# KirillHit/snn_for_object_detection

Hardware: AMD Instinct MI355X
Metric: event-frames/sec (BxT) SODa-3M GEN1 304x240 fwd+bwd (higher is better)
Workload: dtype f32 (16-bit split products)

## Files before the change

include/snn_hip.h:

```cpp
#ifndef SNN_HIP_H
#define SNN_HIP_H

#include <stddef.h>
#include <stdint.h>

#ifdef __cplusplus
extern "C" {
#endif

#define SNN_ABI_VERSION 20

enum {
    SNN_NEURON_NONE = 0,
    SNN_NEURON_LIF = 1,
    SNN_NEURON_LI = 2,
    SNN_NEURON_LI_TANH = 3,
    SNN_NEURON_SLI = 4,
    SNN_NEURON_SYNAPSE = 5
};

enum { SNN_PREC_FP32 = 0, SNN_PREC_BF16X3 = 1, SNN_PREC_BF16X6 = 3, SNN_PREC_FP16X3 = 4, SNN_PREC_BF16X1 = 5,
       SNN_PREC_BF16S = 6 };

enum { SNN_SCAN_WIDE_ADDRESSING = 1,
// ... 95 lines not shown
int snn_conv2d_spikes_wgrad(const float* vdec, int64_t ld, float v_th, const float* dy, int64_t lddy, float* dw, int64_t N,
                            int H, int W, int Cin, int Ho, int Wo, int Cout, int KH, int KW, int stride, int pad,
                            int accumulate, float* workspace, int splitk, void* stream);
int snn_conv3x3_halo_spikes(const float* vdec, int64_t ld, float v_th, const void* w_image, float* y, int64_t ldy, int64_t N,
                            int H, int W, int Cin, int Cout, double* bn_partial, int frames_per_step, int* bn_layout,
                            void* stream);

int snn_conv1x1_mask_supported(int64_t N, int H, int W, int Cin, int Cout, const uint32_t* mask, int64_t ld_mask,
                               const float* w, const float* y, int64_t ldy, const float* dy, int64_t lddy, const float* dw,
                               int fwd_precision, int bwd_precision);
int snn_conv1x1_mask_fwd(const uint32_t* mask, int64_t ld_mask, const float* w, float* y, int64_t ldy, int64_t N, int H, int W,
                         int Cin, int Cout, void* stream);
int snn_conv1x1_mask_wgrad(const uint32_t* mask, int64_t ld_mask, const float* dy, int64_t lddy, float* dw, int64_t N, int H,
                           int W, int Cin, int Cout, int accumulate, float* workspace, int splitk, void* stream);

size_t snn_bn_stats_partial_size(int T, int64_t M, int C);
int snn_bn_stats(const float* y, int64_t ldy, int T, int64_t M, int C, double* partial, void* stream);
int snn_bn_stats_finalize(const double* partial, int chunks, int rows_per_chunk, int T, int64_t M, int C,
                          const float* gamma, const float* bias, float eps, float momentum,
                          float* running_mean, float* running_var, int use_running,
                          float* mean, float* invstd, float* alpha, float* beta, void* stream);

int snn_bn_stats_reduce(const double* partial, int chunks, int rows_per_chunk, int T, int64_t M, int C, double* sums,
                        void* stream);
int snn_bn_stats_from_sums(const double* sums, int T, int64_t M_total, int C,
                           const float* gamma, const float* bias, float eps, float momentum,
                           float* running_mean, float* running_var,
                           float* mean, float* invstd, float* alpha, float* beta,
                           double* var_scratch, void* stream);

// ... 278 lines not shown
```

snn_for_object_detection_amd/_hip.py:

```python

import ctypes
import os
from ctypes import POINTER, Structure, c_char_p, c_double, c_float, c_int, c_int32, c_int64, c_size_t, c_void_p

_HERE = os.path.dirname(os.path.abspath(__file__))
LIB_PATH = os.environ.get("SNN_HIP_LIB") or os.path.join(_HERE, "libsnn_hip.so")

NEURON_NONE, NEURON_LIF, NEURON_LI, NEURON_LI_TANH, NEURON_SLI, NEURON_SYNAPSE = 0, 1, 2, 3, 4, 5
POOL_AVG, POOL_MAX, POOL_SUM = 0, 1, 2
ACT_RELU, ACT_SILU, ACT_TANH = 0, 1, 2
ABI_VERSION = 20
PREC_FP32, PREC_BF16X3, PREC_BF16X6, PREC_FP16X3, PREC_BF16X1, PREC_BF16S = 0, 1, 3, 4, 5, 6
SCAN_WIDE_ADDRESSING, SCAN_LAST_STEP_ONLY, SCAN_BF16_STORAGE, SCAN_SPIKES_FROM_VDEC, SCAN_SUMS_FROM_STATE = 1, 2, 4, 8, 16
SCAN_STATE_LOOKBACK = 32
SCAN_SPIKE_MASK = 32
SURR_SUPER, SURR_TRIANGLE, SURR_SIGMOID, SURR_ATAN = 0, 1, 2, 3
ACTIVITY_NONZERO_F32, ACTIVITY_NONZERO_BF16, ACTIVITY_ABOVE_F32, ACTIVITY_ABOVE_BF16, ACTIVITY_MASK = 0, 1, 2, 3, 4
EVENT_REPS = {"binary": 0, "count": 1, "time": 2, "voxel": 3}
LOSS_CLS_MODES = {"ce": 0, "focal": 1}
LOSS_BOX_MODES = {"l1": 0, "giou": 1, "diou": 2, "ciou": 3}


class NeuronParams(Structure):
    _fields_ = [("c_mem", c_float), ("c_syn", c_float), ("v_leak", c_float), ("v_th", c_float),
# ... 36 lines not shown
    "snn_conv3x3_halo": (c_int, [_P, _L, _P, _P, _L, _L, _I, _I, _I, _I, _P, _L, _P, _L, _P, _I, _P, _I, _P]),
    "snn_conv2d_dgrad": (c_int, [_P, _L, _P, _P, _P, _L, _L, _I, _I, _I, _I, _I, _I, _I, _I, _I, _I, _P, _L, _P, _L,
                                 _I, _P]),
    "snn_conv2d_wgrad": (c_int, [_P, _L, _P, _L, _P, _L, _I, _I, _I, _I, _I, _I, _I, _I, _I, _I, _I, _P, _I, _I,
                                 _P]),
    "snn_conv2d_wgrad_splitk": (c_int, [_L, _I, _I, _I, _I, _I, _I, _I, _I, _I, _I, _I]),
    "snn_conv2d_wgrad_kernel": (c_int, [_L, _I, _I, _I, _I, _I, _I, _I, _I, _I, _I, _I]),
    "snn_conv2d_gather_plan": (c_int, [_I, _L, _I, _I, _I, _I, _I, _I, _I, _I, _I, _I, _L, _L, _I, _I, _I, _I, _I, _I, _I, _P]),
    "snn_conv2d_wgrad_plan": (c_int, [_L, _I, _I, _I, _I, _I, _I, _I, _I, _I, _I, _L, _L, _I, _I, _I, _I, _P]),
    "snn_conv1x1_spikes_supported": (c_int, [_L, _I, _I, _I, _I, _L, _I, _I]),
    "snn_conv1x1_spikes_fwd": (c_int, [_P, _L, _F, _P, _P, _L, _L, _I, _I, _I, _I, _P]),
    "snn_conv1x1_spikes_wgrad": (c_int, [_P, _L, _F, _P, _L, _P, _L, _I, _I, _I, _I, _I, _P, _I, _P]),
    "snn_conv1x1_mask_supported": (c_int, [_L, _I, _I, _I, _I, _P, _L, _P, _P, _L, _P, _L, _P, _I, _I]),
    "snn_conv1x1_mask_fwd": (c_int, [_P, _L, _P, _P, _L, _L, _I, _I, _I, _I, _P]),
    "snn_conv1x1_mask_wgrad": (c_int, [_P, _L, _P, _L, _P, _L, _I, _I, _I, _I, _I, _P, _I, _P]),
    "snn_conv2d_spikes_supported": (c_int, [_L, _I, _I, _I, _I, _I, _I, _I, _I, _I, _I, _L, _I, _I]),
    "snn_conv2d_spikes_fwd": (c_int, [_P, _L, _F, _P, _P, _L, _L, _I, _I, _I, _I, _I, _I, _I, _I, _I, _I, _P, _I, _P, _P]),
    "snn_conv2d_spikes_wgrad": (c_int, [_P, _L, _F, _P, _L, _P, _L, _I, _I, _I, _I, _I, _I, _I, _I, _I, _I, _I, _P, _I, _P]),
    "snn_conv3x3_halo_spikes": (c_int, [_P, _L, _F, _P, _P, _L, _L, _I, _I, _I, _I, _P, _I, _P, _P]),
    "snn_bn_stats_partial_size": (c_size_t, [_I, _L, _I]),
    "snn_bn_stats": (c_int, [_P, _L, _I, _L, _I, _P, _P]),
    "snn_bn_stats_finalize": (c_int, [_P, _I, _I, _I, _L, _I, _P, _P, _F, _F, _P, _P, _I, _P, _P, _P, _P, _P]),
    "snn_bn_stats_reduce": (c_int, [_P, _I, _I, _I, _L, _I, _P, _P]),
    "snn_bn_stats_from_sums": (c_int, [_P, _I, _L, _I, _P, _P, _F, _F, _P, _P, _P, _P, _P, _P, _P, _P]),
    "snn_bn_bwd_reduce": (c_int, [_P, _I, _L, _I, _P, _P]),
    "snn_bn_bwd_coef": (c_int, [_P, _P, _P, _I, _L, _I, _P, _P, _P, _P, _P, _P, _P, _P, _I, _P]),
    "snn_affine_neuron_fwd": (c_int, [_I, _P, _L, _P, _P, _P, _P, _P, _L, _P, _L, _P, _P, _P, _I, _L, _I,
                                      POINTER(NeuronParams), _I, _P]),
    "snn_affine_neuron_fwd_mask": (c_int, [_I, _P, _L, _P, _P, _P, _P, _P, _L, _P, _L, _P, _P, _P, _I, _L, _I,
                                           POINTER(NeuronParams), _I, _P, _P, _L]),
# ... 144 lines not shown
```

snn_for_object_detection_amd/csrc/conv_wgrad.hip:

```cpp
#include <stdlib.h>
#include <type_traits>
#include "conv_common.h"

namespace {

constexpr int WB_K = 32;

struct WgradGeom {
    int64_t Mtot;
    int H, W, Cin, Ho, Wo, Cout, KH, KW, stride, pad;
    int64_t ldx, lddy;
    int Ktot;
    int64_t pix_per_split;
    int tiles_m, tiles_n, splitk;
    int nimg;
    float x_th;
};

template <int TM, int TN, int WM, int WN, bool VEC>
__global__ __launch_bounds__(kThreads, SNN_CONV_MIN_WAVES) void k_conv_wgrad(const float* __restrict__ x, const float* __restrict__ dy,
                                                         float* __restrict__ ws, WgradGeom g) {
    static_assert(WM * WN == 4, "4 waves");
    constexpr int BMc = 32 * TM * WM, BNk = 32 * TN * WN;
    constexpr int DG = BMc / 4, XG = BNk / 4;
// ... 159 lines not shown
    float* slab = ws + (int64_t)z * g.Cout * (int64_t)g.Ktot;
#pragma unroll
    for (int i = 0; i < TM; ++i)
#pragma unroll
        for (int j = 0; j < TN; ++j) {
            const int kc = kc0 + (wn * TN + j) * 32 + r;
            if (kc >= g.Ktot) continue;
#pragma unroll
            for (int e = 0; e < 16; ++e) {
                const int co = co0 + (wm * TM + i) * 32 + (e & 3) + 8 * (e >> 2) + 4 * h;
                if (co < g.Cout) slab[(int64_t)co * g.Ktot + kc] = acc[i][j][e];
            }
        }
}

template <int TM, int TN, int WM, int WN, int WBK, bool ONE, bool SB = false, bool XSP = false, bool XM = false>
__global__ __launch_bounds__(kThreads, 2) void k_conv_wgrad_pipe(const float* __restrict__ x,
                                                                 const float* __restrict__ dy,
                                                                 float* __restrict__ ws, WgradGeom g) {
    static_assert(WM * WN == 4, "4 waves");
    constexpr int BMc = 32 * TM * WM, BNk = 32 * TN * WN;
    constexpr int DG = BMc / 4, XG = BNk / 4;
    static_assert(WBK == 32 || WBK == 64, "stage length");
    static_assert(!SB || ONE, "bf16 storage: one product");
    static_assert(!XSP || (!ONE && !SB), "spikes from potentials: the bf16 x 3 kernel");
    static_assert(!XM || XSP, "spike bit mask: an instance of the spikes-from-potentials kernel");
    constexpr int XW = ((BNk / 32) * WBK + kThreads - 1) / kThreads;
    constexpr int ES = SB ? 2 : 4;
    constexpr int LDW = WBK + 8;
    constexpr int NQ = WBK / 4;
    constexpr int GPP = kThreads / NQ;
    constexpr int DQ = (DG + GPP - 1) / GPP, XQ = (XG + GPP - 1) / GPP;
    __shared__ __attribute__((aligned(16))) __bf16 Dh[BMc * LDW];
    __shared__ __attribute__((aligned(16))) __bf16 Dl[ONE ? 8 : BMc * LDW];
    __shared__ __attribute__((aligned(16))) __bf16 Xh[XM ? 8 : BNk * LDW];
    __shared__ __attribute__((aligned(16))) __bf16 Xl[(ONE || XSP) ? 8 : BNk * LDW];
// ... 192 lines not shown
                for (int c = 0; c < 4; ++c) {
                    *reinterpret_cast<bf16x4*>(&Xh[(x_cq[q] + c) * LDW + quad * 4]) = px[q][c][0];
                    if constexpr (!ONE && !XSP) *reinterpret_cast<bf16x4*>(&Xl[(x_cq[q] + c) * LDW + quad * 4]) = px[q][c][1];
                }
            }
    };

    f32x16 acc[TM][TN];
#pragma unroll
    for (int i = 0; i < TM; ++i)
#pragma unroll
        for (int j = 0; j < TN; ++j)
#pragma unroll
            for (int e = 0; e < 16; ++e) acc[i][j][e] = 0.f;

    auto mfma_group = [&](int ks) {
        bf16x8 ah[TM], al[TM], bh[TN], bl[TN];
#pragma unroll
        for (int i = 0; i < TM; ++i) {
            const int off = ((wm * TM + i) * 32 + r) * LDW + ks * 16 + 8 * h;
            ah[i] = *reinterpret_cast<const bf16x8*>(&Dh[off]);
            if constexpr (!ONE) al[i] = *reinterpret_cast<const bf16x8*>(&Dl[off]);
        }
#pragma unroll
        for (int j = 0; j < TN; ++j) {
            if constexpr (XM) {
                const u32x4 w0 = *reinterpret_cast<const u32x4*>(&Xw[(wn * TN + j) * WBK + ks * 16 + 8 * h]);
                const u32x4 w1 = *reinterpret_cast<const u32x4*>(&Xw[(wn * TN + j) * WBK + ks * 16 + 8 * h + 4]);
                u32x4 d;
                d[0] = (((w0[0] >> r) & 1u) | (((w0[1] >> r) & 1u) << 16)) * 0x3F80u;
// ... 34 lines not shown
    for (int k = 0; k < XW; ++k) pxw[k] = rxw[k];
#pragma unroll
    for (int q = 0; q < XQ; ++q) {
        if constexpr (XM) continue;
        else if constexpr (XSP) convert_spikes(rx[q], px[q]);
        else convert_quad(rx[q], px[q]);
    }
    write_tiles();
    load_tiles(p_lo + WBK, 1);
    decode(0);
    __syncthreads();

    int slot = 0;
#pragma unroll 1
    for (unsigned p0 = p_lo; p0 < p_hi; p0 += WBK) {
        mfma_group(0);
#pragma unroll
        for (int q = 0; q < DQ; ++q) convert_quad(rd[q], pd[q]);
        __builtin_amdgcn_sched_group_barrier(0x100, NREAD, 0);
#pragma unroll
        for (int m = 0; m < NM; ++m) {
            __builtin_amdgcn_sched_group_barrier(0x008, 1, 0);
            __builtin_amdgcn_sched_group_barrier(0x002, VPG_D, 0);
        }
        __builtin_amdgcn_sched_barrier(0);
        mfma_group(1);
#pragma unroll
        for (int k = 0; k < XW; ++k) pxw[k] = rxw[k];
#pragma unroll
        for (int q = 0; q < XQ; ++q) {
            if constexpr (XM) continue;
            else if constexpr (XSP) convert_spikes(rx[q], px[q]);
            else convert_quad(rx[q], px[q]);
        }
        __builtin_amdgcn_sched_group_barrier(0x100, NREAD, 0);
#pragma unroll
        for (int m = 0; m < NM; ++m) {
            __builtin_amdgcn_sched_group_barrier(0x008, 1, 0);
            __builtin_amdgcn_sched_group_barrier(0x002, VPG_X, 0);
        }
        __builtin_amdgcn_sched_barrier(0);
#pragma unroll
        for (int ks = 2; ks < WBK / 16; ++ks) mfma_group(ks);
        load_tiles(p0 + 2 * WBK, slot);
        __syncthreads();
        write_tiles();
        decode(slot ^ 1);
        __syncthreads();
        slot ^= 1;
    }

    float* slab = ws + (int64_t)z * g.Cout * (int64_t)g.Ktot;
#pragma unroll
    for (int i = 0; i < TM; ++i)
#pragma unroll
        for (int j = 0; j < TN; ++j) {
            const int kcol = kc0 + (wn * TN + j) * 32 + r;
            if (kcol >= g.Ktot) continue;
// ... 392 lines not shown
    g.pix_per_split = p.pix_per_split;
    g.nimg = (int)N;
    g.tiles_m = p.tiles_m;
    g.tiles_n = p.tiles_n;
    g.splitk = splitk;
    dim3 grid((unsigned)((int64_t)g.tiles_m * g.tiles_n * splitk));
    hipStream_t st = (hipStream_t)stream;
    dispatch(
        [&](auto ID, auto KERNEL, auto WBK, auto ONE, auto SB, auto XSP, auto XM) {
            constexpr WgradShape t = kWgradShapes[ID()];
            if constexpr (KERNEL() != kWgradPipe) {
                hipLaunchKernelGGL((k_conv_wgrad<t.tm, t.tn, t.wm, t.wn, KERNEL() == kWgradVec>), grid, dim3(kThreads), 0, st, x, dy,
                                   workspace, g);
            } else if constexpr ((!SB() || ONE()) && (!XSP() || (!ONE() && !SB())) && (!XM() || XSP())) {
                hipLaunchKernelGGL((k_conv_wgrad_pipe<t.tm, t.tn, t.wm, t.wn, WBK(), ONE(), SB(), XSP(), XM()>), grid, dim3(kThreads), 0,
                                   st, x, dy, workspace, g);
            }
            return true;
        },
        OneOf<0, 1, 2, 3, 4, 5>{p.t.id}, OneOf<0, 1, 2>{p.kernel}, OneOf<32, 64>{p.wbk}, Flag{p.one}, Flag{sbf}, Flag{xsp}, Flag{xm});
    SNN_CHECK_LAUNCH("snn_conv2d_wgrad");
    return wgrad_reduce_slabs(workspace, dw, (int64_t)Cout * g.Ktot, splitk, accumulate, st);
}

extern "C" int snn_conv2d_wgrad_splitk(int64_t N, int H, int W, int Cin, int Ho, int Wo, int Cout, int KH, int KW,
                                       int stride, int pad, int precision) {
    if (N <= 0 || Ho <= 0 || Wo <= 0 || Cin <= 0 || Cout <= 0 || KH <= 0 || KW <= 0) return 1;
    return wgrad_plan(N, H, W, Cin, Ho, Wo, Cout, KH, KW, stride, pad, Cin, Cout, kAlignAll, precision, false, 0, 0).splitk;
}

extern "C" int snn_conv2d_wgrad_kernel(int64_t N, int H, int W, int Cin, int Ho, int Wo, int Cout, int KH, int KW, int stride,
// ... 88 lines not shown
        return false;
    const unsigned align = kAlignIn16 | kAlignDy16 | kAlignDy8 | (aligned(16, {dw}) ? kAlignDw16 : 0u);
    const WgradPlan p = wgrad_plan(N, H, W, Cin, H, W, Cout, 1, 1, 1, 0, ld_mask, lddy, align, SNN_PREC_BF16X3, true, 0, 0, false, true);
    return p.ok && p.kernel == kWgradPipe;
}

extern "C" int snn_conv1x1_mask_wgrad(const uint32_t* mask, int64_t ld_mask, const float* dy, int64_t lddy, float* dw, int64_t N,
                                      int H, int W, int Cin, int Cout, int accumulate, float* workspace, int splitk,
                                      void* stream) {
    SNN_REQUIRE(mask && dy && dw && workspace, "snn_conv1x1_mask_wgrad: null pointer");
    SNN_REQUIRE(snn_wgrad_mask_ok(N, H, W, Cin, Cout, mask, ld_mask, dy, lddy, dw),
                "snn_conv1x1_mask_wgrad: call not covered (ask snn_conv1x1_mask_supported)");
    return wgrad_common(reinterpret_cast<const float*>(mask), ld_mask, dy, lddy, dw, N, H, W, Cin, H, W, Cout, 1, 1, 1, 0,
                        accumulate, workspace, splitk, SNN_PREC_BF16X3, stream, true, 0.0f, true);
}
```

snn_for_object_detection_amd/functional.py:

```python

import collections
import contextlib
import ctypes
import functools
import os
import struct
from typing import List, NamedTuple, Optional, Sequence, Tuple

import torch
from torch.autograd import Function

from . import _hip
from ._hip import NeuronParams
from ._layout import (_BF16, _F32, ConcatPromise, Dest, _add_cl, _alias, _cl_view, _Convert, _copy_cl,
                      _dims5, _new_cl, _out_tensor, _ptr, _raw_convert, _raw_dense_cl, _raw_to_cl, _raw_to_nchw,
                      _require_device, _stream, _through_fp32, _ToChannelsLast, as_sequence, cl_stride, is_channels_last,
                      to_bfloat16, to_channels_last, to_float32)
from .pointwise import (POOL2D_COVERED, _Act, _Pool, _PoolPad, _SPP, _Upsample, activation, pool2d,
                        pool_covers, pool_sets, spp_covers, upsample_nearest)
from .losses import (MAX_LABEL_STEPS, _DetectionLoss, _GatherSteps, _loss_entry, _loss_ext, _require_steps,
                     check_loss_options, detection_loss, detection_loss_ext, detection_loss_steps,
                     detection_loss_steps_ext, gather_steps, select_label_steps)
from .event_ops import (AUG_Q16_MAX, AUG_Q16_MIN, AUG_Q16_ONE, _check_batch_vectors, _launch_batch_scatter,
                        check_aug_table, events_to_frames, events_to_frames_aug, events_to_frames_packed, labels_augment)

LEVERS = ("USE_WGRAD_STREAM", "USE_HEAD_STREAMS", "WGRAD_SIDE_DEPTH", "FUSE_OUTER_ADDEND", "USE_SIBLING_FUSION",
          "USE_SPIKES_FROM_VDEC", "USE_SPIKE_MASK", "SPIKE_MASK_MIN_BYTES", "USE_HALO_CONV", "USE_DEFERRED_BN_APPLY",
          "SCAN_SEGMENT_T", "USE_CONV_BN_STATS", "USE_PRESPLIT_WEIGHTS", "USE_PRESPLIT_DGRAD", "SCAN_FLAGS",
          "USE_SUMS_FROM_STATE", "LIF_CHECKPOINT_BYTES", "USE_LSTM_SCAN")


@contextlib.contextmanager
def levers(**values):
    unknown = sorted(set(values) - set(LEVERS))
    if unknown:
        raise AttributeError(f"functional has no lever {', '.join(unknown)} (LEVERS: {', '.join(LEVERS)})")
    found = {name: globals()[name] for name in values}
    globals().update(values)
    try:
        yield
    finally:
        globals().update(found)

DEFAULT_DT = 0.001
# ... 385 lines not shown
        self.result = dx


def _acc_of(x):
    return getattr(x, "_snn_acc", None)


def _same_tensor(a: torch.Tensor, b: torch.Tensor) -> bool:
    return (a.data_ptr() == b.data_ptr() and tuple(a.shape) == tuple(b.shape) and a.stride() == b.stride())


def _slot_of(param) -> Optional[GradSlot]:
    return getattr(param, "_snn_grad_slot", None) if param is not None else None


def _dgrad_accumulate(acc, gy, ldg, wt, x, geom, st, prec, wt_split=None, wt_image=None):
    T, B, Cin, H, W, Cout, KH, KW, Ho, Wo, stride, pad = geom
    dx, dx_shape = None, (T, B, Cin, H, W)
    addend, ld_add, addend2, ld_add2 = None, 0, None, 0
    outer_fused = None
    if acc is not None and acc[0].result is None and acc[0].deposits:
        key, other = next(iter(acc[0].deposits.items()))
        other = _raw_to_cl(other)
        if tuple(other.shape) == dx_shape:
            addend, ld_add = other.data_ptr(), cl_stride(other)
            acc[0].fused[key] = acc[0].deposits.pop(key)
    if (acc is not None and acc[0].result is None and not acc[0].deposits and acc[0].outer is not None
            and FUSE_OUTER_ADDEND):
        o_acc, o_key = acc[0].outer
        if o_acc.result is None and len(o_acc.deposits) == 1 and o_key not in o_acc.deposits:
            key2, other2 = next(iter(o_acc.deposits.items()))
            other2 = _raw_to_cl(other2)
            if tuple(other2.shape) == dx_shape:
                addend2, ld_add2 = other2.data_ptr(), cl_stride(other2)
                outer_fused = (o_acc, o_key, key2)
                if (o_acc.grad_in_slot and key2 in o_acc.exclusive and other2.dtype == x.dtype and ld_add2 % 4 == 0
                        and USE_SIBLING_FUSION):
                    dx = _alias(other2, other2.storage_offset(), T, B, Cin, H, W, ld_add2)
    chained = False
    if (acc is not None and acc[0].result is not None and addend is None and acc[1] not in acc[0].fused
            and tuple(acc[0].result.shape) == dx_shape):
        prev = acc[0].result
        addend, ld_add = prev.data_ptr(), cl_stride(prev)
        chained = True
    if dx is None:
        dx = _new_cl((T, B), Cin, H, W, x)
    if (prec in _HALO_BWD_PRECS and _halo_operand_ok(gy.data_ptr(), ldg, prec == _hip.PREC_BF16S) and USE_HALO_CONV
            and (KH, KW, stride, pad) == (3, 3, 2, 1)
            and _hip.query("snn_conv3x3_s2_dgrad_supported", T * B, H, W, Cin, Ho, Wo, Cout)):
        if wt_image is None:
            wt_image = _frag_image(wt, Cin, Cout, 1, _hip.PREC_BF16X3)
        _hip.call("snn_conv3x3_s2_dgrad", gy.data_ptr(), ldg, wt_image.data_ptr(), dx.data_ptr(), cl_stride(dx), T * B, H, W, Cin, Ho,
                  Wo, Cout, addend, ld_add, addend2, ld_add2, prec, st)
    elif (prec in _HALO_BWD_PRECS and _halo_operand_ok(gy.data_ptr(), ldg, prec == _hip.PREC_BF16S)
            and _halo_ok(T * B, H, W, Cout, Cin, KH, KW, stride, pad)):
        if wt_image is None:
            wt_image = _frag_image(wt, Cin, Cout, 1, _hip.PREC_BF16X3)
        _hip.call("snn_conv3x3_halo", gy.data_ptr(), ldg, wt_image.data_ptr(), dx.data_ptr(), cl_stride(dx), T * B, H, W, Cout,
                  Cin, addend, ld_add, addend2, ld_add2, None, 0, None, prec, st)
    else:
        _hip.call("snn_conv2d_dgrad", gy.data_ptr(), ldg, wt.data_ptr(), wt_split, dx.data_ptr(), cl_stride(dx), T * B, H, W,
                  Cin, Ho, Wo, Cout, KH, KW, stride, pad, addend, ld_add, addend2, ld_add2, prec, st)
    if acc is not None and (acc[0].result is None or chained):
        if chained and acc[0].outer is not None and acc[0].outer[0].result is acc[0].result:
            acc[0].outer[0].set_result(dx)
            acc[0].outer[0].fused[acc[0].outer[1]] = dx
        acc[0].set_result(dx)
        acc[0].fused[acc[1]] = dx
    if outer_fused is not None:
        o_acc, o_key, key2 = outer_fused
        o_acc.fused[key2] = o_acc.deposits.pop(key2)
        o_acc.fused[o_key] = dx
        o_acc.set_result(dx)
    return dx


USE_HALO_CONV = not os.environ.get("SNN_NO_HALO_CONV")
_HALO_BWD_PRECS = (_hip.PREC_BF16X3, _hip.PREC_BF16S)


def _halo_ok(N: int, H: int, W: int, Cin: int, Cout: int, KH: int, KW: int, stride: int, pad: int) -> bool:
    return (USE_HALO_CONV and KH == 3 and KW == 3 and stride == 1 and pad == 1
            and bool(_hip.query("snn_conv3x3_halo_supported", N, H, W, Cin, Cout)))


def _halo_operand_ok(ptr: int, ld: int, bf16: bool) -> bool:
    return ld % 4 == 0 and ptr % (8 if bf16 else 16) == 0


# ... 142 lines not shown
        dx = dw = None
        pend = _PENDING_APPLY.pop(gy.data_ptr(), None)
        if pend is not None:
            fused = (not ctx.needs_input_grad[0] and ctx.needs_input_grad[1] and ctx.slot is not None
                     and pend.gx.dtype == _F32 and pend.dims == (T, B, Cout, Ho, Wo) and cl_stride(pend.y) % 4 == 0
                     and _hip.query("snn_conv2d_wgrad_bn_supported", T * B, H, W, Cin, Ho, Wo, Cout, KH, KW, stride, pad))
            if fused:
                splitk = _hip.query("snn_conv2d_wgrad_splitk", T * B, H, W, Cin, Ho, Wo, Cout, KH, KW, stride, pad, ctx.prec)
                with _WgradLaunch(x.device, True, splitk, Cout, KH * KW * Cin,
                                   hold=(x, pend.gx, pend.y, pend.coef)) as (stream, ws, _):
                    _hip.call("snn_conv2d_wgrad_bn", x.data_ptr(), ldx, pend.gx.data_ptr(), Cout, pend.y.data_ptr(),
                              cl_stride(pend.y), pend.coef.data_ptr(), T, B, ctx.slot.buf.data_ptr(), T * B, H, W, Cin, Ho,
                              Wo, Cout, KH, KW, stride, pad, ctx.slot.claim(), ws.data_ptr(), splitk, stream)
                return None, None, None, None, None, None, None, None, None, None
            _apply_pending(pend)
        if ctx.needs_input_grad[0]:
            wt = _kept_view(ctx.weight, "_snn_wt")
            wt16 = wt_img = None
            if wt is not None:
                wt_img = _kept_view(ctx.weight, "_snn_wtfrag")
                if ctx.prec == _hip.PREC_BF16X3 and USE_PRESPLIT_WEIGHTS and USE_PRESPLIT_DGRAD:
                    wt16 = _ptr(_kept_view(ctx.weight, "_snn_wt16"))
            else:
                wt = torch.empty((Cin, KH, KW, Cout), device=x.device, dtype=_F32)
                _hip.call("snn_weight_transpose", w_ohwi.data_ptr(), wt.data_ptr(), Cout, KH, KW, Cin, st)
            dx = _dgrad_accumulate(ctx.acc, gy, ldg, wt, x, ctx.geom, st, ctx.prec, wt_split=wt16, wt_image=wt_img)
        if ctx.needs_input_grad[1]:
            splitk = _hip.query("snn_conv2d_wgrad_splitk", T * B, H, W, Cin, Ho, Wo, Cout, KH, KW, stride, pad, ctx.prec)
            xw, ldxw, x_th = _spikes_wgrad_operand(x, ldx, ctx.x_th, gy, ldg)
            slot = ctx.slot
            with _WgradLaunch(x.device, slot is not None, splitk, Cout, KH * KW * Cin,
                              hold=(x, xw, gy)) as (stream, ws, _):
                if slot is not None:
                    dst, accumulate = slot.buf, slot.claim()
                else:
                    dst, accumulate = torch.empty((Cout, KH, KW, Cin), device=x.device, dtype=_F32), 0
                if x_th is not None:
                    _hip.call("snn_conv2d_spikes_wgrad", xw.data_ptr(), ldxw, x_th, gy.data_ptr(), ldg, dst.data_ptr(),
                              T * B, H, W, Cin, Ho, Wo, Cout, KH, KW, stride, pad, accumulate, ws.data_ptr(), splitk,
                              stream)
                else:
                    _hip.call("snn_conv2d_wgrad", xw.data_ptr(), ldxw, gy.data_ptr(), ldg, dst.data_ptr(), T * B, H, W,
                              Cin, Ho, Wo, Cout, KH, KW, stride, pad, accumulate, ws.data_ptr(), splitk, ctx.prec,
                              stream)
            if slot is None:
                dw = dst.permute(0, 3, 1, 2)
        return dx, dw, None, None, None, None, None, None, None, None


def _small_gemm(a: torch.Tensor, trans_a: bool, b: torch.Tensor, trans_b: bool, c: torch.Tensor, accumulate: int,
                ct: Optional[torch.Tensor] = None, ct_col: int = 0) -> None:
    m, n = c.shape
# ... 144 lines not shown
        ctx.widths, ctx.c1 = widths, C1
        ctx.slot1, ctx.slots2 = slot1, slots2
        ctx.acc = acc
        return y

    @staticmethod
    def backward(ctx, gy):
        x, w1m, *w2ms = ctx.saved_tensors
        T, B, Cin, H, W, Ct = ctx.geom[:6]
        C1, widths = ctx.c1, ctx.widths
        composed = w1m is not None
        gy = _raw_to_cl(gy)
        ldg, ldx = cl_stride(gy), cl_stride(x)
        dx = dw1 = None
        dw2s = [None] * len(widths)
        if ctx.needs_input_grad[0]:
            dx = _dgrad_accumulate(ctx.acc, gy, ldg, ctx.wct, x, ctx.geom, _stream(), ctx.prec)
        if any(ctx.needs_input_grad[9:]) or (composed and ctx.needs_input_grad[1]):
            slot1, slots2 = ctx.slot1, ctx.slots2
            slotted = all(s_ is not None for s_ in slots2) and (slot1 is not None or not composed)
            splitk = _hip.query("snn_conv2d_wgrad_splitk", T * B, H, W, Cin, H, W, Ct, 1, 1, 1, 0, ctx.prec)
            xw, ldxw, x_th = _spikes_wgrad_operand(x, ldx, ctx.x_th, gy, ldg)
            x_mask = ctx.x_mask
            with _WgradLaunch(x.device, slotted, splitk, Ct, Cin, hold=(x, xw, gy, x_mask), with_g=True) as (stream, ws, G):
                if x_mask is not None and _hip.query("snn_conv1x1_mask_supported", T * B, H, W, Cin, Ct, x_mask.data_ptr(),
                                                     x_mask.shape[-1], None, None, 0, gy.data_ptr(), ldg, G.data_ptr(),
                                                     ctx.fwd_prec, ctx.prec):
                    _hip.call("snn_conv1x1_mask_wgrad", x_mask.data_ptr(), x_mask.shape[-1], gy.data_ptr(), ldg, G.data_ptr(),
                              T * B, H, W, Cin, Ct, 0, ws.data_ptr(), splitk, stream)
                elif x_th is not None:
                    _hip.call("snn_conv1x1_spikes_wgrad", xw.data_ptr(), ldxw, x_th, gy.data_ptr(), ldg, G.data_ptr(),
                              T * B, H, W, Cin, Ct, 0, ws.data_ptr(), splitk, stream)
                else:
                    _hip.call("snn_conv2d_wgrad", xw.data_ptr(), ldxw, gy.data_ptr(), ldg, G.data_ptr(), T * B, H, W,
                              Cin, H, W, Ct, 1, 1, 1, 0, 0, ws.data_ptr(), splitk, ctx.prec, stream)
                g1 = None
                if composed:
                    g1 = slot1.buf.view(C1, Cin) if slotted else torch.empty((C1, Cin), device=x.device, dtype=_F32)
                    acc1 = slot1.claim() if slotted else 0
                row = 0
                for b, (w2m, c) in enumerate(zip(w2ms, widths)):
                    Gb = G[row:row + c]
# ... 1139 lines not shown
```

snn_for_object_detection_amd/profiler.py:

```python

from collections import defaultdict
from typing import Dict

import torch


WGRAD_LABELS = ("k_conv_wgrad_pipe", "k_conv_wgrad_halo", "k_conv_first<wgrad>")


def _wgrad_label(n, h, w, cin, ho, wo, cout, kh, kw, stride, pad, prec) -> str:
    from . import _hip
    return WGRAD_LABELS[int(_hip.query("snn_conv2d_wgrad_kernel", n, h, w, cin, ho, wo, cout, kh, kw, stride, pad, prec))]


def _conv_label(name: str, a) -> str:
    if name == "snn_conv2d_wgrad":
        return _wgrad_label(a[5], a[6], a[7], a[8], a[9], a[10], a[11], a[12], a[13], a[14], a[15], a[19])
    dgrad = name == "snn_conv2d_dgrad"
    cin, cout = a[8], a[11]
    oc, ic = (cin, cout) if dgrad else (cout, cin)
    if not dgrad and cin == 2 and a[12] == 3 and a[13] == 3 and cout % 4 == 0 and (cout // 4) & (cout // 4 - 1) == 0 \
            and cout <= 256 and a[16] is None:
        return "k_conv_first<2, 3, false>"
    if oc <= 32:
# ... 31 lines not shown
        flops = 2.0 * n * h * w * cout * cin
        byts = 4.0 * (n * h * w * cin + n * h * w * cout + cout * cin)
        if not fwd:
            return WGRAD_LABELS[0], flops, byts
        tile = "32, 4, 1" if cout <= 32 else ("64, 2, 2" if cout <= 64 else "128, 2, 2")
        return f"k_conv_gather<{tile}, false, true>", flops, byts
    if name in ("snn_conv1x1_mask_fwd", "snn_conv1x1_mask_wgrad"):
        fwd = name.endswith("_fwd")
        n, h, w, cin, cout = (a[5], a[6], a[7], a[8], a[9])
        flops = 2.0 * n * h * w * cout * cin
        byts = n * h * w * cin / 8.0 + 4.0 * (n * h * w * cout + cout * cin)
        if not fwd:
            return WGRAD_LABELS[0] + ", mask, spikes", flops, byts
        tile = "32, 4, 1" if cout <= 32 else ("64, 2, 2" if cout <= 64 else "128, 2, 2")
        return f"k_conv_gather<{tile}, false, true>, mask, spikes", flops, byts
    if name in ("snn_conv2d_spikes_fwd", "snn_conv2d_spikes_wgrad"):
        fwd = name.endswith("_fwd")
        n, h, w, cin, ho, wo, cout, kh, kw, stride, pad = a[6:17]
        flops = 2.0 * n * ho * wo * cout * kh * kw * cin
        byts = 4.0 * (n * h * w * cin + n * ho * wo * cout + cout * kh * kw * cin)
        if not fwd:
            return _wgrad_label(n, h, w, cin, ho, wo, cout, kh, kw, stride, pad, 1) + ", spikes", flops, byts
        tile = "32, 4, 1" if cout <= 32 else ("64, 2, 2" if cout <= 64 else "128, 2, 2")
        return f"k_conv_gather<{tile}, false, true>", flops, byts
    if name == "snn_conv3x3_halo_spikes":
        n, h, w, cin, cout = a[6], a[7], a[8], a[9], a[10]
        flops = 2.0 * n * h * w * cout * 9 * cin
        byts = 4.0 * (n * h * w * cin + n * h * w * cout) + 4.0 * cout * 9 * cin
        return f"k_conv_halo3<{128 if cout % 128 == 0 else (64 if cout % 64 == 0 else 32)}, fwd, spikes>", flops, byts
    if name == "snn_conv3x3_halo":
# ... 123 lines not shown
```

Before: 7431.

## Fuse 1x1 conv data gradient into pipelined weight-gradient kernel

Adds a DX variant of the pipelined bf16x3 weight-gradient kernel. It reuses the dy tiles already staged in LDS (read transposed via ds_read_tr16) to compute dx for 1x1 convolutions, with the weights split into high and low bf16 parts held in registers, and it adds optional addends. The Python backward paths for plain and composed 1x1 convs route through this fused call when eligible, then run only a split-k reduce for dw. The goal is to avoid a separate dgrad pass that re-reads dy, at the cost of higher register pressure (launch bounds drop to 1 for some tiles) and extra MFMA work inside the wgrad loop.

New measurement: 7524, median of 6. 1.2% higher.

```diff
diff --git a/include/snn_hip.h b/include/snn_hip.h
--- a/include/snn_hip.h
+++ b/include/snn_hip.h
@@ -133,6 +133,20 @@
 int snn_conv1x1_mask_wgrad(const uint32_t* mask, int64_t ld_mask, const float* dy, int64_t lddy, float* dw, int64_t N, int H,
                            int W, int Cin, int Cout, int accumulate, float* workspace, int splitk, void* stream);
 
+int snn_conv1x1_bwd_supported(int64_t N, int H, int W, int Cin, int Cout, const void* x, int64_t ldx, int is_mask,
+                              const float* dy, int64_t lddy, const float* wt, const float* dx, int64_t lddx,
+                              const float* addend, int64_t ld_addend, const float* addend2, int64_t ld_addend2,
+                              const float* dw, int splitk, int precision);
+int snn_conv1x1_bwd(const float* x, int64_t ldx, const float* dy, int64_t lddy, const float* wt, float* dx, int64_t lddx,
+                    const float* addend, int64_t ld_addend, const float* addend2, int64_t ld_addend2, float* dw, int64_t N,
+                    int H, int W, int Cin, int Cout, int accumulate, float* workspace, int splitk, int precision,
+                    void* stream);
+int snn_conv1x1_mask_bwd(const uint32_t* mask, int64_t ld_mask, const float* dy, int64_t lddy, const float* wt, float* dx,
+                         int64_t lddx, const float* addend, int64_t ld_addend, const float* addend2, int64_t ld_addend2,
+                         float* dw, int64_t N, int H, int W, int Cin, int Cout, int accumulate, float* workspace, int splitk,
+                         int precision, void* stream);
+int snn_conv2d_wgrad_reduce(float* workspace, float* dw, int64_t n, int splitk, int accumulate, void* stream);
+
 size_t snn_bn_stats_partial_size(int T, int64_t M, int C);
 int snn_bn_stats(const float* y, int64_t ldy, int T, int64_t M, int C, double* partial, void* stream);
 int snn_bn_stats_finalize(const double* partial, int chunks, int rows_per_chunk, int T, int64_t M, int C,
diff --git a/snn_for_object_detection_amd/_hip.py b/snn_for_object_detection_amd/_hip.py
--- a/snn_for_object_detection_amd/_hip.py
+++ b/snn_for_object_detection_amd/_hip.py
@@ -74,6 +74,10 @@
     "snn_conv1x1_mask_supported": (c_int, [_L, _I, _I, _I, _I, _P, _L, _P, _P, _L, _P, _L, _P, _I, _I]),
     "snn_conv1x1_mask_fwd": (c_int, [_P, _L, _P, _P, _L, _L, _I, _I, _I, _I, _P]),
     "snn_conv1x1_mask_wgrad": (c_int, [_P, _L, _P, _L, _P, _L, _I, _I, _I, _I, _I, _P, _I, _P]),
+    "snn_conv1x1_bwd_supported": (c_int, [_L, _I, _I, _I, _I, _P, _L, _I, _P, _L, _P, _P, _L, _P, _L, _P, _L, _P, _I, _I]),
+    "snn_conv1x1_bwd": (c_int, [_P, _L, _P, _L, _P, _P, _L, _P, _L, _P, _L, _P, _L, _I, _I, _I, _I, _I, _P, _I, _I, _P]),
+    "snn_conv1x1_mask_bwd": (c_int, [_P, _L, _P, _L, _P, _P, _L, _P, _L, _P, _L, _P, _L, _I, _I, _I, _I, _I, _P, _I, _I, _P]),
+    "snn_conv2d_wgrad_reduce": (c_int, [_P, _P, _L, _I, _I, _P]),
     "snn_conv2d_spikes_supported": (c_int, [_L, _I, _I, _I, _I, _I, _I, _I, _I, _I, _I, _L, _I, _I]),
     "snn_conv2d_spikes_fwd": (c_int, [_P, _L, _F, _P, _P, _L, _L, _I, _I, _I, _I, _I, _I, _I, _I, _I, _I, _P, _I, _P, _P]),
     "snn_conv2d_spikes_wgrad": (c_int, [_P, _L, _F, _P, _L, _P, _L, _I, _I, _I, _I, _I, _I, _I, _I, _I, _I, _I, _P, _I, _P]),
diff --git a/snn_for_object_detection_amd/csrc/conv_wgrad.hip b/snn_for_object_detection_amd/csrc/conv_wgrad.hip
--- a/snn_for_object_detection_amd/csrc/conv_wgrad.hip
+++ b/snn_for_object_detection_amd/csrc/conv_wgrad.hip
@@ -197,12 +197,22 @@
         }
 }
 
-template <int TM, int TN, int WM, int WN, int WBK, bool ONE, bool SB = false, bool XSP = false, bool XM = false>
-__global__ __launch_bounds__(kThreads, 2) void k_conv_wgrad_pipe(const float* __restrict__ x,
+struct WgradDx {
+    const float* wt;
+    float* dx;
+    const float* add1;
+    const float* add2;
+    int64_t lddx, ld_add1, ld_add2;
+};
+typedef short s16x4 __attribute__((ext_vector_type(4)));
+template <int TM, int TN, int WM, int WN, int WBK, bool ONE, bool SB = false, bool XSP = false, bool XM = false, bool DX = false>
+__global__ __launch_bounds__(kThreads, (DX && TM * TN == 4 && !XM) ? 1 : 2) void k_conv_wgrad_pipe(const float* __restrict__ x,
                                                                  const float* __restrict__ dy,
-                                                                 float* __restrict__ ws, WgradGeom g) {
+                                                                 float* __restrict__ ws, WgradGeom g, WgradDx d) {
     static_assert(WM * WN == 4, "4 waves");
     constexpr int BMc = 32 * TM * WM, BNk = 32 * TN * WN;
+    static_assert(!DX || (!ONE && !SB && XSP == XM), "fused data gradient: bf16 x 3 on fp32 x or on the spike bit mask");
+    static_assert(!DX || (BNk / 32) * (WBK / 32) == 4, "fused data gradient: one 32 x 32 dx tile per wave and stage");
     constexpr int DG = BMc / 4, XG = BNk / 4;
     static_assert(WBK == 32 || WBK == 64, "stage length");
     static_assert(!SB || ONE, "bf16 storage: one product");
@@ -425,6 +435,36 @@
 #pragma unroll
             for (int e = 0; e < 16; ++e) acc[i][j][e] = 0.f;
 
+    constexpr int NCH = BMc / 16;
+    [[maybe_unused]] bf16x8 wh[DX ? NCH : 1], wl[DX ? NCH : 1];
+    [[maybe_unused]] const int dx_cg = wave % (BNk / 32), dx_pg = wave / (BNk / 32);
+    [[maybe_unused]] int dx_tr = 0;
+    if constexpr (DX) {
+        const int ci = kc0 + dx_cg * 32 + r;
+#pragma unroll
+        for (int c = 0; c < NCH; ++c) {
+            const int co = 16 * c + 8 * h;
+            f32x4 v[2] = {{0.f, 0.f, 0.f, 0.f}, {0.f, 0.f, 0.f, 0.f}};
+            if (ci < g.Cin) {
+                if (co < g.Cout) v[0] = *reinterpret_cast<const f32x4*>(d.wt + (int64_t)ci * g.Cout + co);
+                if (co + 4 < g.Cout) v[1] = *reinterpret_cast<const f32x4*>(d.wt + (int64_t)ci * g.Cout + co + 4);
+            }
+#pragma unroll
+            for (int e = 0; e < 8; e += 2) {
+                f32x2 rest = {v[e >> 2][e & 3], v[e >> 2][(e & 3) + 1]};
+                bf16x2 pp = __builtin_convertvector(rest, bf16x2);
+                const unsigned bits = __builtin_bit_cast(unsigned, pp);
+                wh[c][e] = pp[0]; wh[c][e + 1] = pp[1];
+                rest[0] -= __builtin_bit_cast(float, bits << 16);
+                rest[1] -= __builtin_bit_cast(float, bits & 0xffff0000u);
+                pp = __builtin_convertvector(rest, bf16x2);
+                wl[c][e] = pp[0]; wl[c][e + 1] = pp[1];
+            }
+        }
+        const int grp = lane_id >> 4, i16 = lane_id & 15;
+        dx_tr = (8 * (grp >> 1) + (i16 >> 2)) * LDW + dx_pg * 32 + 16 * (grp & 1) + 4 * (i16 & 3);
+    }
+
     auto mfma_group = [&](int ks) {
         bf16x8 ah[TM], al[TM], bh[TN], bl[TN];
 #pragma unroll
@@ -489,6 +529,18 @@
     int slot = 0;
 #pragma unroll 1
     for (unsigned p0 = p_lo; p0 < p_hi; p0 += WBK) {
+        [[maybe_unused]] f32x4 ad1[4], ad2[4];
+        [[maybe_unused]] const unsigned dx_p = p0 + (unsigned)(dx_pg * 32 + r);
+        [[maybe_unused]] const int dx_ci = kc0 + dx_cg * 32 + 4 * h;
+        if constexpr (DX) {
+#pragma unroll
+            for (int jj = 0; jj < 4; ++jj) {
+                const bool ok = dx_p < p_hi && dx_ci + 8 * jj < g.Cin;
+                ad1[jj] = ad2[jj] = f32x4{0.f, 0.f, 0.f, 0.f};
+                if (d.add1 && ok) ad1[jj] = SnnStore<false>::ld4_last(d.add1, (int64_t)dx_p * d.ld_add1 + dx_ci + 8 * jj);
+                if (d.add2 && ok) ad2[jj] = SnnStore<false>::ld4_last(d.add2, (int64_t)dx_p * d.ld_add2 + dx_ci + 8 * jj);
+            }
+        }
         mfma_group(0);
 #pragma unroll
         for (int q = 0; q < DQ; ++q) convert_quad(rd[q], pd[q]);
@@ -517,6 +569,33 @@
         __builtin_amdgcn_sched_barrier(0);
 #pragma unroll
         for (int ks = 2; ks < WBK / 16; ++ks) mfma_group(ks);
+        if constexpr (DX) {
+            f32x16 dacc;
+#pragma unroll
+            for (int e = 0; e < 16; ++e) dacc[e] = 0.f;
+            typedef __attribute__((address_space(3))) s16x4* LdsQuad;
+#pragma unroll
+            for (int c = 0; c < NCH; ++c) {
+                const int o = dx_tr + 16 * c * LDW;
+                const s16x4 h0 = __builtin_amdgcn_ds_read_tr16_b64_v4i16((LdsQuad)&Dh[o]);
+                const s16x4 h1 = __builtin_amdgcn_ds_read_tr16_b64_v4i16((LdsQuad)&Dh[o + 4 * LDW]);
+                const s16x4 l0 = __builtin_amdgcn_ds_read_tr16_b64_v4i16((LdsQuad)&Dl[o]);
+                const s16x4 l1 = __builtin_amdgcn_ds_read_tr16_b64_v4i16((LdsQuad)&Dl[o + 4 * LDW]);
+                const bf16x8 dh = __builtin_bit_cast(bf16x8, __builtin_shufflevector(h0, h1, 0, 1, 2, 3, 4, 5, 6, 7));
+                const bf16x8 dl = __builtin_bit_cast(bf16x8, __builtin_shufflevector(l0, l1, 0, 1, 2, 3, 4, 5, 6, 7));
+                dacc = __builtin_amdgcn_mfma_f32_32x32x16_bf16(wh[c], dl, dacc, 0, 0, 0);
+                dacc = __builtin_amdgcn_mfma_f32_32x32x16_bf16(wl[c], dh, dacc, 0, 0, 0);
+                dacc = __builtin_amdgcn_mfma_f32_32x32x16_bf16(wh[c], dh, dacc, 0, 0, 0);
+            }
+#pragma unroll
+            for (int jj = 0; jj < 4; ++jj) {
+                if (!(dx_p < p_hi && dx_ci + 8 * jj < g.Cin)) continue;
+                f32x4 v = {dacc[4 * jj], dacc[4 * jj + 1], dacc[4 * jj + 2], dacc[4 * jj + 3]};
+                if (d.add1) v += ad1[jj];
+                if (d.add2) v += ad2[jj];
+                SnnStore<false>::st4(d.dx, (int64_t)dx_p * d.lddx + dx_ci + 8 * jj, v);
+            }
+        }
         load_tiles(p0 + 2 * WBK, slot);
         __syncthreads();
         write_tiles();
@@ -939,7 +1018,7 @@
                                    workspace, g);
             } else if constexpr ((!SB() || ONE()) && (!XSP() || (!ONE() && !SB())) && (!XM() || XSP())) {
                 hipLaunchKernelGGL((k_conv_wgrad_pipe<t.tm, t.tn, t.wm, t.wn, WBK(), ONE(), SB(), XSP(), XM()>), grid, dim3(kThreads), 0,
-                                   st, x, dy, workspace, g);
+                                   st, x, dy, workspace, g, WgradDx{});
             }
             return true;
         },
@@ -1058,3 +1137,116 @@
     return wgrad_common(reinterpret_cast<const float*>(mask), ld_mask, dy, lddy, dw, N, H, W, Cin, H, W, Cout, 1, 1, 1, 0,
                         accumulate, workspace, splitk, SNN_PREC_BF16X3, stream, true, 0.0f, true);
 }
+
+namespace {
+struct Bwd1x1Call {
+    const void* x;
+    int64_t ldx;
+    bool xm;
+    const float* dy;
+    int64_t lddy;
+    const float* wt;
+    const float* dx;
+    int64_t lddx;
+    const float *add1, *add2;
+    int64_t ld_add1, ld_add2;
+    const float* dw;
+};
+static const char* bwd1x1_refusal(int64_t N, int H, int W, int Cin, int Cout, const Bwd1x1Call& c, int splitk, int precision,
+                                  WgradPlan* out) {
+    if (!(N > 0 && H > 0 && W > 0 && Cin > 0 && Cout > 0)) return "bad shape";
+    if (!(c.x && c.dy && c.wt && c.dx)) return "null pointer";
+    if (precision != SNN_PREC_BF16X3) return "bf16 x 3 arithmetic on fp32 tensors only";
+    if (Cout > 128) return "more than 128 output channels (a block must own all of them)";
+    if (Cout % 4 || Cin % 4) return "channel counts must be multiples of 4";
+    if (splitk < 0 || splitk > 32768) return "bad splitk";
+    if (c.xm ? !(Cin % 32 == 0 && c.ldx >= Cin / 32) : !(c.ldx >= Cin && c.ldx % 4 == 0))
+        return "x: pixel stride smaller than the channel count or no multiple of 4 (mask: Cin % 32, ld >= Cin / 32)";
+    if (!(c.lddy >= Cout && c.lddy % 4 == 0 && c.lddx >= Cin && c.lddx % 4 == 0))
+        return "dy / dx: pixel stride smaller than the channel count or no multiple of 4";
+    if (!(aligned(c.xm ? 4 : 16, {c.x}) && aligned(16, {c.dy, c.wt, c.dx}))) return "x, dy, wt and dx must be 16-byte aligned (mask: 4)";
+    if (c.add1 && !(c.ld_add1 >= Cin && c.ld_add1 % 4 == 0 && aligned(16, {c.add1}))) return "addend: stride or alignment";
+    if (c.add2 && !(c.ld_add2 >= Cin && c.ld_add2 % 4 == 0 && aligned(16, {c.add2}))) return "addend2: stride or alignment";
+    if (c.dw && !aligned(4, {c.dw})) return "dw must be 4-byte aligned";
+    if (!(N * H * (int64_t)W < 0x7fffffffLL - 64)) return "more than 2^31 pixels";
+    const unsigned align = kAlignIn16 | kAlignDy16 | kAlignDy8 | ((c.dw && aligned(16, {c.dw})) ? kAlignDw16 : 0u);
+    const WgradPlan p = wgrad_plan(N, H, W, Cin, H, W, Cout, 1, 1, 1, 0, c.ldx, c.lddy, align, precision, c.xm, 0, splitk, false, c.xm);
+    if (!(p.ok && p.kernel == kWgradPipe && !p.one)) return "the weight gradient does not take the pipelined bf16 x 3 kernel";
+    if (p.tiles_m != 1) return "the weight-gradient tile does not own all output channels";
+    if (!(p.t.id == 0 || p.t.id == 4)) return "no fused instance for this weight-gradient tile";
+    if (out) *out = p;
+    return nullptr;
+}
+
+static bool bwd1x1_pays(const WgradPlan& p, bool xm) {
+    return !(p.t.id == 0 && !xm);
+}
+
+static int bwd1x1_common(const char* name, const Bwd1x1Call& c, float* dx, float* dw, int64_t N, int H, int W, int Cin, int Cout,
+                         int accumulate, float* workspace, int splitk, int precision, void* stream) {
+    SNN_REQUIRE(workspace, "%s: null workspace", name);
+    SNN_REQUIRE(splitk >= 1, "%s: bad splitk %d", name, splitk);
+    WgradPlan p;
+    const char* why = bwd1x1_refusal(N, H, W, Cin, Cout, c, splitk, precision, &p);
+    SNN_REQUIRE(!why, "%s: call not covered: %s (ask snn_conv1x1_bwd_supported)", name, why);
+    WgradGeom g;
+    g.Mtot = N * H * (int64_t)W;
+    g.H = H; g.W = W; g.Cin = Cin; g.Ho = H; g.Wo = W; g.Cout = Cout;
+    g.KH = 1; g.KW = 1; g.stride = 1; g.pad = 0;
+    g.ldx = c.ldx; g.lddy = c.lddy;
+    g.Ktot = Cin;
+    g.x_th = 0.0f;
+    g.pix_per_split = p.pix_per_split;
+    g.nimg = (int)N;
+    g.tiles_m = p.tiles_m;
+    g.tiles_n = p.tiles_n;
+    g.splitk = splitk;
+    const WgradDx d = {c.wt, dx, c.add1, c.add2, c.lddx, c.ld_add1, c.ld_add2};
+    const dim3 grid((unsigned)((int64_t)g.tiles_m * g.tiles_n * splitk));
+    hipStream_t st = (hipStream_t)stream;
+    const float* xf = static_cast<const float*>(c.x);
+    dispatch(
+        [&](auto ID, auto XM) {
+            constexpr WgradShape t = kWgradShapes[ID()];
+            constexpr int wbk = ID() >= 4 ? 64 : 32;
+            hipLaunchKernelGGL((k_conv_wgrad_pipe<t.tm, t.tn, t.wm, t.wn, wbk, false, false, XM(), XM(), true>), grid, dim3(kThreads), 0, st,
+                               xf, c.dy, workspace, g, d);
+            return true;
+        },
+        OneOf<0, 4>{p.t.id}, Flag{c.xm});
+    SNN_CHECK_LAUNCH(name);
+    if (!dw) return 0;
+    return wgrad_reduce_slabs(workspace, dw, (int64_t)Cout * Cin, splitk, accumulate, st);
+}
+}
+
+extern "C" int snn_conv1x1_bwd_supported(int64_t N, int H, int W, int Cin, int Cout, const void* x, int64_t ldx, int is_mask,
+                                         const float* dy, int64_t lddy, const float* wt, const float* dx, int64_t lddx,
+                                         const float* addend, int64_t ld_addend, const float* addend2, int64_t ld_addend2,
+                                         const float* dw, int splitk, int precision) {
+    const Bwd1x1Call c = {x, ldx, is_mask != 0, dy, lddy, wt, dx, lddx, addend, addend2, ld_addend, ld_addend2, dw};
+    WgradPlan p;
+    if (bwd1x1_refusal(N, H, W, Cin, Cout, c, splitk, precision, &p)) return 0;
+    return bwd1x1_pays(p, c.xm) ? 1 : 0;
+}
+
+extern "C" int snn_conv1x1_bwd(const float* x, int64_t ldx, const float* dy, int64_t lddy, const float* wt, float* dx, int64_t lddx,
+                               const float* addend, int64_t ld_addend, const float* addend2, int64_t ld_addend2, float* dw,
+                               int64_t N, int H, int W, int Cin, int Cout, int accumulate, float* workspace, int splitk,
+                               int precision, void* stream) {
+    const Bwd1x1Call c = {x, ldx, false, dy, lddy, wt, dx, lddx, addend, addend2, ld_addend, ld_addend2, dw};
+    return bwd1x1_common("snn_conv1x1_bwd", c, dx, dw, N, H, W, Cin, Cout, accumulate, workspace, splitk, precision, stream);
+}
+
+extern "C" int snn_conv1x1_mask_bwd(const uint32_t* mask, int64_t ld_mask, const float* dy, int64_t lddy, const float* wt, float* dx,
+                                    int64_t lddx, const float* addend, int64_t ld_addend, const float* addend2,
+                                    int64_t ld_addend2, float* dw, int64_t N, int H, int W, int Cin, int Cout, int accumulate,
+                                    float* workspace, int splitk, int precision, void* stream) {
+    const Bwd1x1Call c = {mask, ld_mask, true, dy, lddy, wt, dx, lddx, addend, addend2, ld_addend, ld_addend2, dw};
+    return bwd1x1_common("snn_conv1x1_mask_bwd", c, dx, dw, N, H, W, Cin, Cout, accumulate, workspace, splitk, precision, stream);
+}
+
+extern "C" int snn_conv2d_wgrad_reduce(float* workspace, float* dw, int64_t n, int splitk, int accumulate, void* stream) {
+    SNN_REQUIRE(workspace && dw && n > 0 && splitk >= 1 && splitk <= 32768, "snn_conv2d_wgrad_reduce: bad arguments");
+    return wgrad_reduce_slabs(workspace, dw, n, splitk, accumulate, (hipStream_t)stream);
+}
diff --git a/snn_for_object_detection_amd/functional.py b/snn_for_object_detection_amd/functional.py
--- a/snn_for_object_detection_amd/functional.py
+++ b/snn_for_object_detection_amd/functional.py
@@ -27,7 +27,8 @@
 LEVERS = ("USE_WGRAD_STREAM", "USE_HEAD_STREAMS", "WGRAD_SIDE_DEPTH", "FUSE_OUTER_ADDEND", "USE_SIBLING_FUSION",
           "USE_SPIKES_FROM_VDEC", "USE_SPIKE_MASK", "SPIKE_MASK_MIN_BYTES", "USE_HALO_CONV", "USE_DEFERRED_BN_APPLY",
           "SCAN_SEGMENT_T", "USE_CONV_BN_STATS", "USE_PRESPLIT_WEIGHTS", "USE_PRESPLIT_DGRAD", "SCAN_FLAGS",
-          "USE_SUMS_FROM_STATE", "LIF_CHECKPOINT_BYTES", "USE_LSTM_SCAN")
+          "USE_SUMS_FROM_STATE", "LIF_CHECKPOINT_BYTES", "USE_LSTM_SCAN", "USE_FUSED_BWD1X1",
+          "FUSED_BWD1X1_MIN_BYTES")
 
 
 @contextlib.contextmanager
@@ -443,7 +444,7 @@
     return getattr(param, "_snn_grad_slot", None) if param is not None else None
 
 
-def _dgrad_accumulate(acc, gy, ldg, wt, x, geom, st, prec, wt_split=None, wt_image=None):
+def _dgrad_accumulate(acc, gy, ldg, wt, x, geom, st, prec, wt_split=None, wt_image=None, fuse=None):
     T, B, Cin, H, W, Cout, KH, KW, Ho, Wo, stride, pad = geom
     dx, dx_shape = None, (T, B, Cin, H, W)
     addend, ld_add, addend2, ld_add2 = None, 0, None, 0
@@ -474,7 +475,9 @@
         chained = True
     if dx is None:
         dx = _new_cl((T, B), Cin, H, W, x)
-    if (prec in _HALO_BWD_PRECS and _halo_operand_ok(gy.data_ptr(), ldg, prec == _hip.PREC_BF16S) and USE_HALO_CONV
+    if fuse is not None and fuse(dx, addend, ld_add, addend2, ld_add2):
+        pass
+    elif (prec in _HALO_BWD_PRECS and _halo_operand_ok(gy.data_ptr(), ldg, prec == _hip.PREC_BF16S) and USE_HALO_CONV
             and (KH, KW, stride, pad) == (3, 3, 2, 1)
             and _hip.query("snn_conv3x3_s2_dgrad_supported", T * B, H, W, Cin, Ho, Wo, Cout)):
         if wt_image is None:
@@ -502,6 +505,36 @@
         o_acc.fused[o_key] = dx
         o_acc.set_result(dx)
     return dx
+
+
+USE_FUSED_BWD1X1 = not os.environ.get("SNN_NO_FUSED_BWD1X1")
+FUSED_BWD1X1_MIN_BYTES = 4 << 20
+
+
+class _FusedBwd1x1:
+
+    __slots__ = ("gy", "ldg", "wt", "xop", "ldxop", "is_mask", "geom", "prec", "splitk", "ws")
+
+    def __init__(self, gy, ldg, wt, xop, ldxop, is_mask, geom, prec, splitk):
+        self.gy, self.ldg, self.wt, self.xop, self.ldxop, self.is_mask = gy, ldg, wt, xop, ldxop, is_mask
+        self.geom, self.prec, self.splitk, self.ws = geom, prec, splitk, None
+
+    @staticmethod
+    def eligible(geom, prec, gy, x) -> bool:
+        T, B, _, H, W, Cout = geom[:6]
+        return (USE_FUSED_BWD1X1 and tuple(geom[6:8]) == (1, 1) and tuple(geom[10:12]) == (1, 0)
+                and T * B * H * W * Cout * 4 >= FUSED_BWD1X1_MIN_BYTES and prec == _hip.PREC_BF16X3 and gy.dtype == _F32 and x.dtype == _F32)
+
+    def __call__(self, dx, addend, ld_add, addend2, ld_add2) -> bool:
+        T, B, Cin, H, W, Cout = self.geom[:6]
+        tail = (self.gy.data_ptr(), self.ldg, self.wt.data_ptr(), dx.data_ptr(), cl_stride(dx), addend, ld_add, addend2, ld_add2)
+        if not _hip.query("snn_conv1x1_bwd_supported", T * B, H, W, Cin, Cout, self.xop.data_ptr(), self.ldxop,
+                          int(self.is_mask), *tail, None, self.splitk, self.prec):
+            return False
+        self.ws = torch.empty((self.splitk, Cout * Cin), device=dx.device, dtype=_F32)
+        _hip.call("snn_conv1x1_mask_bwd" if self.is_mask else "snn_conv1x1_bwd", self.xop.data_ptr(), self.ldxop, *tail, None,
+                  T * B, H, W, Cin, Cout, 0, self.ws.data_ptr(), self.splitk, self.prec, _stream())
+        return True
 
 
 USE_HALO_CONV = not os.environ.get("SNN_NO_HALO_CONV")
@@ -674,6 +707,7 @@
                               Wo, Cout, KH, KW, stride, pad, ctx.slot.claim(), ws.data_ptr(), splitk, stream)
                 return None, None, None, None, None, None, None, None, None, None
             _apply_pending(pend)
+        fuse = None
         if ctx.needs_input_grad[0]:
             wt = _kept_view(ctx.weight, "_snn_wt")
             wt16 = wt_img = None
@@ -684,18 +718,24 @@
             else:
                 wt = torch.empty((Cin, KH, KW, Cout), device=x.device, dtype=_F32)
                 _hip.call("snn_weight_transpose", w_ohwi.data_ptr(), wt.data_ptr(), Cout, KH, KW, Cin, st)
-            dx = _dgrad_accumulate(ctx.acc, gy, ldg, wt, x, ctx.geom, st, ctx.prec, wt_split=wt16, wt_image=wt_img)
+            if ctx.needs_input_grad[1] and ctx.x_th is None and _FusedBwd1x1.eligible(ctx.geom, ctx.prec, gy, x):
+                fuse = _FusedBwd1x1(gy, ldg, wt, x, ldx, False, ctx.geom, ctx.prec, _hip.query(
+                    "snn_conv2d_wgrad_splitk", T * B, H, W, Cin, Ho, Wo, Cout, KH, KW, stride, pad, ctx.prec))
+            dx = _dgrad_accumulate(ctx.acc, gy, ldg, wt, x, ctx.geom, st, ctx.prec, wt_split=wt16, wt_image=wt_img, fuse=fuse)
         if ctx.needs_input_grad[1]:
             splitk = _hip.query("snn_conv2d_wgrad_splitk", T * B, H, W, Cin, Ho, Wo, Cout, KH, KW, stride, pad, ctx.prec)
             xw, ldxw, x_th = _spikes_wgrad_operand(x, ldx, ctx.x_th, gy, ldg)
             slot = ctx.slot
-            with _WgradLaunch(x.device, slot is not None, splitk, Cout, KH * KW * Cin,
-                              hold=(x, xw, gy)) as (stream, ws, _):
+            fws = fuse.ws if fuse is not None else None
+            with _WgradLaunch(x.device, slot is not None, 0 if fws is not None else splitk, Cout, KH * KW * Cin,
+                              hold=(x, xw, gy, fws)) as (stream, ws, _):
                 if slot is not None:
                     dst, accumulate = slot.buf, slot.claim()
                 else:
                     dst, accumulate = torch.empty((Cout, KH, KW, Cin), device=x.device, dtype=_F32), 0
-                if x_th is not None:
+                if fws is not None:
+                    _hip.call("snn_conv2d_wgrad_reduce", fws.data_ptr(), dst.data_ptr(), Cout * Cin, splitk, accumulate, stream)
+                elif x_th is not None:
                     _hip.call("snn_conv2d_spikes_wgrad", xw.data_ptr(), ldxw, x_th, gy.data_ptr(), ldg, dst.data_ptr(),
                               T * B, H, W, Cin, Ho, Wo, Cout, KH, KW, stride, pad, accumulate, ws.data_ptr(), splitk,
                               stream)
@@ -870,18 +910,30 @@
         ldg, ldx = cl_stride(gy), cl_stride(x)
         dx = dw1 = None
         dw2s = [None] * len(widths)
+        want_dw = any(ctx.needs_input_grad[9:]) or (composed and ctx.needs_input_grad[1])
+        fuse = None
         if ctx.needs_input_grad[0]:
-            dx = _dgrad_accumulate(ctx.acc, gy, ldg, ctx.wct, x, ctx.geom, _stream(), ctx.prec)
-        if any(ctx.needs_input_grad[9:]) or (composed and ctx.needs_input_grad[1]):
+            if want_dw and _FusedBwd1x1.eligible(ctx.geom, ctx.prec, gy, x) and (ctx.x_th is None or ctx.x_mask is not None):
+                splitk = _hip.query("snn_conv2d_wgrad_splitk", T * B, H, W, Cin, H, W, Ct, 1, 1, 1, 0, ctx.prec)
+                if ctx.x_mask is None:
+                    fuse = _FusedBwd1x1(gy, ldg, ctx.wct, x, ldx, False, ctx.geom, ctx.prec, splitk)
+                else:
+                    fuse = _FusedBwd1x1(gy, ldg, ctx.wct, ctx.x_mask, ctx.x_mask.shape[-1], True, ctx.geom, ctx.prec, splitk)
+            dx = _dgrad_accumulate(ctx.acc, gy, ldg, ctx.wct, x, ctx.geom, _stream(), ctx.prec, fuse=fuse)
+        if want_dw:
             slot1, slots2 = ctx.slot1, ctx.slots2
             slotted = all(s_ is not None for s_ in slots2) and (slot1 is not None or not composed)
             splitk = _hip.query("snn_conv2d_wgrad_splitk", T * B, H, W, Cin, H, W, Ct, 1, 1, 1, 0, ctx.prec)
             xw, ldxw, x_th = _spikes_wgrad_operand(x, ldx, ctx.x_th, gy, ldg)
             x_mask = ctx.x_mask
-            with _WgradLaunch(x.device, slotted, splitk, Ct, Cin, hold=(x, xw, gy, x_mask), with_g=True) as (stream, ws, G):
-                if x_mask is not None and _hip.query("snn_conv1x1_mask_supported", T * B, H, W, Cin, Ct, x_mask.data_ptr(),
-                                                     x_mask.shape[-1], None, None, 0, gy.data_ptr(), ldg, G.data_ptr(),
-                                                     ctx.fwd_prec, ctx.prec):
+            fws = fuse.ws if fuse is not None else None
+            with _WgradLaunch(x.device, slotted, 0 if fws is not None else splitk, Ct, Cin, hold=(x, xw, gy, x_mask, fws),
+                              with_g=True) as (stream, ws, G):
+                if fws is not None:
+                    _hip.call("snn_conv2d_wgrad_reduce", fws.data_ptr(), G.data_ptr(), Ct * Cin, splitk, 0, stream)
+                elif x_mask is not None and _hip.query("snn_conv1x1_mask_supported", T * B, H, W, Cin, Ct, x_mask.data_ptr(),
+                                                       x_mask.shape[-1], None, None, 0, gy.data_ptr(), ldg, G.data_ptr(),
+                                                       ctx.fwd_prec, ctx.prec):
                     _hip.call("snn_conv1x1_mask_wgrad", x_mask.data_ptr(), x_mask.shape[-1], gy.data_ptr(), ldg, G.data_ptr(),
                               T * B, H, W, Cin, Ct, 0, ws.data_ptr(), splitk, stream)
                 elif x_th is not None:
diff --git a/snn_for_object_detection_amd/profiler.py b/snn_for_object_detection_amd/profiler.py
--- a/snn_for_object_detection_amd/profiler.py
+++ b/snn_for_object_detection_amd/profiler.py
@@ -69,6 +69,14 @@
             return WGRAD_LABELS[0] + ", mask, spikes", flops, byts
         tile = "32, 4, 1" if cout <= 32 else ("64, 2, 2" if cout <= 64 else "128, 2, 2")
         return f"k_conv_gather<{tile}, false, true>, mask, spikes", flops, byts
+    if name in ("snn_conv1x1_bwd", "snn_conv1x1_mask_bwd"):
+        mask = name == "snn_conv1x1_mask_bwd"
+        n, h, w, cin, cout = a[12:17]
+        px = float(n) * h * w
+        flops = 4.0 * px * cout * cin
+        addends = (a[7] is not None) + (a[9] is not None)
+        byts = 4.0 * px * cout + (px * cin / 8.0 if mask else 4.0 * px * cin) + 4.0 * px * cin * (1 + addends) + 8.0 * cout * cin
+        return WGRAD_LABELS[0] + ", dgrad+wgrad" + (", mask, spikes" if mask else ""), flops, byts
     if name in ("snn_conv2d_spikes_fwd", "snn_conv2d_spikes_wgrad"):
         fwd = name.endswith("_fwd")
         n, h, w, cin, ho, wo, cout, kh, kw, stride, pad = a[6:17]
```
